# openai/procgen

Hardware: NVIDIA H100
Metric: env-steps/sec (higher is better)
Workload: dtype f32+u8

## Files before the change

procgen_b200/csrc/pg_kernels.cuh:

```cuda
#pragma once
#include "pg_raster.cuh"

namespace pg {

struct KParams {
    EnvHdr *hdr;
    Entity *ents;
    int16_t *grid;
    MT19937 *rng;
    MT19937 *lvl_rng;
    int32_t *scratch;
    RotBlit *rot_scratch;
    Blit *blit_list;
    unsigned char *frame_setup;
    Blit *cell_spill;
    const GameAssets *assets;
    const uint32_t *atlas;
    TileTable tiles;
    const int32_t *action;
    uint8_t *rgb;
    float *rew;
    uint8_t *first;
    int32_t *info_prev_level_seed;
    uint8_t *info_prev_level_complete;
// ... 115 lines not shown
}

template <class G, class Setup>
PG_HD void env_setup_frame(const KParams &p, int env, Setup &f, int lane, int nlanes) {
    Ctx c = make_ctx(p, env);
    using R = Raster<G, Setup>;
    R::setup_frame(c, f, p.snap != 0, lane, nlanes);
#if defined(__CUDA_ARCH__)
    __syncwarp();
#endif
    R::build_entity_blits(c, f, lane, nlanes);
#if defined(__CUDA_ARCH__)
    __syncwarp();
#endif
    if (f.n_jobs > 0) {
        R::frame_tiles(c, f, lane, nlanes);
#if defined(__CUDA_ARCH__)
        __syncwarp();
#endif
    }
    if (G::DEFER_ROTATED) {
        R::frame_rots(c, f, lane, nlanes);
#if defined(__CUDA_ARCH__)
        __syncwarp();
#endif
    }
    if (lane == 0)
        R::frame_append_overlays(f);
    if (G::DRAWS_GRID) {
#if defined(__CUDA_ARCH__)
        __syncwarp();
#endif
        R::frame_build(c, f, lane, nlanes, 0);
#if defined(__CUDA_ARCH__)
        __syncwarp();
#endif
        R::frame_tile_alloc(c, f, p.tiles, lane, nlanes);
#if defined(__CUDA_ARCH__)
        __syncwarp();
#endif
        R::frame_cells_finish(c, f, lane, nlanes);
    } else {
        R::frame_build(c, f, lane, nlanes, 0);
    }
}

template <class Frame>
PG_HD void env_stage_tiles_serial(const KParams &p, Frame &f) {
    const int nj = f.n_tjobs < MAX_TILE_JOBS ? f.n_tjobs : MAX_TILE_JOBS;
    for (int j = 0; j < nj; j++)
        for (int w = 0; w < (int)f.tjob_words[j]; w++) f.arena[f.tjob_dst[j] + w] = p.tiles.texels[f.tjob_src[j] + w];
}

template <class G, class Frame>
PG_HD void env_render_compose(const KParams &p, Frame &f, int row_first, int row_step, int lane, int nlanes) {
    Raster<G, Frame>::compose_rows(f, f.fb, row_first, row_step, lane, nlanes, p.atlas);
}

PG_HD void tile_table_fill(const SpriteDesc *sprites, const uint32_t *index, uint32_t *texels, const uint32_t *atlas, int slot, int tw, int th, int tid,
                           int nthreads) {
    Blit b;
    make_image_blit(b, 0.0, 0.0, (double)tw, (double)th, sprites[slot], false, 256, true);
    uint32_t *dst = texels + index[(slot * MAX_TILE_DIM + (tw - 1)) * MAX_TILE_DIM + (th - 1)];
    const int words = tile_words(tw, th);
    for (int i = tid; i < words; i += nthreads) {
        const int dy = i / tw, dx = i - dy * tw;
        dst[i] = dy < th ? tile_texel(b, atlas, dx, dy) : 0u;
    }
}

template <class G, int VIEW = G::MAX_VIEW_CELLS>
struct FrameFor {
    using type = FrameT<(G::DRAWS_GRID ? VIEW : 1), G::MAX_VISIBLE_ENTS, G::MAX_ROT_BLITS>;
    using setup = FrameSetupT<(G::DRAWS_GRID ? VIEW : 1), G::MAX_VISIBLE_ENTS, G::MAX_ROT_BLITS>;
    using shared = typename type::Shared;
};

}
```

procgen_b200/csrc/pg_launch.cuh:

```cuda
#pragma once
#include <stdarg.h>
#include <stdio.h>
#include <stdlib.h>
#include <string.h>

#include "pg_kernels.cuh"

#ifndef PG_HOSTSIM
#include <cuda_runtime.h>
#endif

namespace pg {

static inline void pg_fatal(const char *fmt, ...) {
    fprintf(stderr, "fatal: ");
    va_list args;
    va_start(args, fmt);
    vfprintf(stderr, fmt, args);
    va_end(args);
    exit(EXIT_FAILURE);
}
#define pg_fassert(cond)                                                                  \
    do {                                                                                  \
        if (!(cond)) {                                                                    \
// ... 104 lines not shown
    }
}
__device__ __forceinline__ void pg_bulk_load(void *dst_smem, const void *src_gmem, unsigned bytes, unsigned long long *bar) {
    asm volatile("cp.async.bulk.shared::cluster.global.mbarrier::complete_tx::bytes [%0], [%1], %2, [%3];" ::"r"(pg_smem_addr(dst_smem)),
                 "l"(src_gmem), "r"(bytes), "r"(pg_smem_addr(bar))
                 : "memory");
}
__device__ __forceinline__ void pg_bulk_store_and_wait(void *dst_gmem, const void *src_smem, unsigned bytes) {
    asm volatile("cp.async.bulk.global.shared::cta.bulk_group [%0], [%1], %2;" ::"l"(dst_gmem), "r"(pg_smem_addr(src_smem)), "r"(bytes) : "memory");
    asm volatile("cp.async.bulk.commit_group;" ::: "memory");
    asm volatile("cp.async.bulk.wait_group.read 0;" ::: "memory");
}

template <class G, int VIEW>
__global__ void __launch_bounds__(kRenderThreads, RenderTune<G, VIEW>::kMinBlocks) render_kernel(KParams p) {
    using Frame = typename FrameFor<G, VIEW>::type;
    extern __shared__ __align__(128) unsigned char smem_raw[];
    Frame &f = *reinterpret_cast<Frame *>(smem_raw);
    const int env = p.env_first + (int)blockIdx.x * p.env_step;
    const int tid = (int)threadIdx.x;
#ifdef PG_PHASE_TIMING
    long long t0 = clock64(), t1;
#define PG_RENDER_PHASE(id)                                       \
    do {                                                          \
        t1 = clock64();                                           \
        if (tid == 0)                                             \
            p.hdr[env].dbg_phase[id] = (uint32_t)(t1 - t0);       \
        t0 = t1;                                                  \
    } while (0)
#else
#define PG_RENDER_PHASE(id) do { } while (0)
#endif
    using Shared = typename FrameFor<G, VIEW>::shared;
    using Setup = typename FrameFor<G, VIEW>::setup;
    const Setup *gs = reinterpret_cast<const Setup *>(p.frame_setup + (size_t)env * p.frame_setup_stride);
    if (tid == 0)
        pg_mbar_init(&f.mbar, 1);
    __syncthreads();
    if (tid < 32) {
        const int nj = G::DRAWS_GRID ? (gs->n_tjobs < MAX_TILE_JOBS ? gs->n_tjobs : MAX_TILE_JOBS) : 0;
        unsigned words = 0;
        for (int j = tid; j < nj; j += 32) words += gs->tjob_words[j];
        for (int d = 16; d > 0; d >>= 1) words += __shfl_xor_sync(0xffffffffu, words, d);
        if (tid == 0) {
            pg_mbar_arrive_expect_tx(&f.mbar, (unsigned)sizeof(Shared) + 4u * words);
            pg_bulk_load(static_cast<Shared *>(&f), static_cast<const Shared *>(gs), (unsigned)sizeof(Shared), &f.mbar);
        }
        __syncwarp();
        for (int j = tid; j < nj; j += 32)
            pg_bulk_load(f.arena + gs->tjob_dst[j], p.tiles.texels + gs->tjob_src[j], 4u * gs->tjob_words[j], &f.mbar);
    }
    pg_mbar_wait(&f.mbar, 0);
    PG_RENDER_PHASE(0);
    env_render_compose<G, Frame>(p, f, tid >> 5, kRenderThreads >> 5, tid & 31, 32);
    __syncthreads();
    PG_RENDER_PHASE(5);
    if (p.consumer != nullptr) {
        const int kf = p.consumer_k, s = p.consumer_slot;
        const int slots = kf == 1 ? 1 : 2 * kf;
        uint32_t *base = reinterpret_cast<uint32_t *>(p.consumer) + (size_t)env * slots * (3 * RES_W * RES_H / 2);
        const uint16_t *lut = p.consumer_lut;
        for (int pair = tid; pair < RES_W * RES_H / 2; pair += kRenderThreads) {
            const uint32_t c0 = f.fb[2 * pair], c1 = f.fb[2 * pair + 1];
#pragma unroll
            for (int ch = 0; ch < 3; ch++) {
                const int sh = 16 - 8 * ch;
                const uint32_t v = (uint32_t)lut[(c0 >> sh) & 0xffu] | ((uint32_t)lut[(c1 >> sh) & 0xffu] << 16);
                base[(size_t)(s * 3 + ch) * (RES_W * RES_H / 2) + pair] = v;
                if (kf > 1)
                    base[(size_t)((s + kf) * 3 + ch) * (RES_W * RES_H / 2) + pair] = v;
            }
        }
        if (kf > 1 && p.first[env]) {
            for (int j = 1; j < kf; j++) {
                const int a = (s + j) % kf;
                for (int w = tid; w < 3 * RES_W * RES_H / 2; w += kRenderThreads) {
                    base[(size_t)a * (3 * RES_W * RES_H / 2) + w] = 0u;
                    base[(size_t)(a + kf) * (3 * RES_W * RES_H / 2) + w] = 0u;
                }
            }
        }
    }
    {
        constexpr int kQuadsPerThread = RES_W * RES_H / 4 / kRenderThreads;
        uint32_t c[kQuadsPerThread][4];
#pragma unroll
        for (int j = 0; j < kQuadsPerThread; j++) {
            const uint4 v = reinterpret_cast<const uint4 *>(f.fb)[tid + j * kRenderThreads];
            c[j][0] = v.x; c[j][1] = v.y; c[j][2] = v.z; c[j][3] = v.w;
        }
        __syncthreads();
#pragma unroll
        for (int j = 0; j < kQuadsPerThread; j++) Raster<G, Frame>::pack_quad(c[j], f.fb + 3 * (tid + j * kRenderThreads));
    }
    asm volatile("fence.proxy.async.shared::cta;" ::: "memory");
    __syncthreads();
    PG_RENDER_PHASE(6);
    if (tid == 0)
        pg_bulk_store_and_wait(p.rgb + (size_t)env * (RES_W * RES_H * 3), f.fb, RES_W * RES_H * 3);
    PG_RENDER_PHASE(7);
#undef PG_RENDER_PHASE
}

#endif

#ifndef PG_HOSTSIM
template <class G>
__global__ void camera_kernel(KParams p) {
    using Frame = typename FrameFor<G>::type;
    if (threadIdx.x == 0 && blockIdx.x < (unsigned)p.env_count) {
        const int env = p.env_first + (int)blockIdx.x * p.env_step;
        Ctx c = make_ctx(p, env);
        Raster<G, Frame>::prepare_camera(c);
        write_step_outputs(p, env, *c.h);
    }
}
#endif

template <class G, int VIEW, class Frame>
void render_env_serial(const KParams &p, int env, Frame &f) {
    using Setup = typename FrameFor<G, VIEW>::setup;
    using Shared = typename FrameFor<G, VIEW>::shared;
    Setup &s = *reinterpret_cast<Setup *>(p.frame_setup + (size_t)env * p.frame_setup_stride);
    env_setup_frame<G, Setup>(p, env, s, 0, 1);
    static_cast<Shared &>(f) = static_cast<const Shared &>(s);
    env_stage_tiles_serial<Frame>(p, f);
    for (int w = 0; w < 4; w++) env_render_compose<G, Frame>(p, f, w, 4, 0, 1);
    uint32_t *out = reinterpret_cast<uint32_t *>(p.rgb + (size_t)env * (RES_W * RES_H * 3));
    for (int g = 0; g < RES_W * RES_H / 4; g++) Raster<G, Frame>::pack_quad(f.fb + 4 * g, out + 3 * g);
}

struct LaunchCtx {
#ifndef PG_HOSTSIM
    cudaStream_t stream;
    cudaStream_t logic_stream;
    cudaEvent_t link;
    unsigned int *ticket;
    int max_logic_blocks;
    int render_smem_floor;
    cudaEvent_t *tev;
#endif
    int64_t *launch_counter;
};

#ifndef PG_HOSTSIM
template <class G, int VIEW>
int prepare_render_smem(const LaunchCtx &lc) {
    using Frame = typename FrameFor<G, VIEW>::type;
    const int bytes = (int)sizeof(Frame) > lc.render_smem_floor ? (int)sizeof(Frame) : lc.render_smem_floor;
    static int attr_set[64] = {};
    int dev = 0;
    CUDA_CHECK(cudaGetDevice(&dev));
    int &have = attr_set[dev & 63];
    if (have < bytes) {
        CUDA_CHECK(cudaFuncSetAttribute(render_kernel<G, VIEW>, cudaFuncAttributeMaxDynamicSharedMemorySize, bytes));
        have = bytes;
    }
    return bytes;
}
#endif

template <class G, bool INIT, int VIEW>
void launch_env_kernel(const KParams &p, const LaunchCtx &lc) {
    using Frame = typename FrameFor<G, VIEW>::type;
    if (p.env_count <= 0)
        return;
#ifndef PG_HOSTSIM
    const int render_smem = prepare_render_smem<G, VIEW>(lc);
    int logic_blocks = (p.env_count + kLogicEnvsPerBlock - 1) / kLogicEnvsPerBlock;
    if (logic_blocks > lc.max_logic_blocks)
        logic_blocks = lc.max_logic_blocks;
    cudaStream_t ls = lc.logic_stream ? lc.logic_stream : lc.stream;
    CUDA_CHECK(cudaMemsetAsync(lc.ticket, 0, sizeof(unsigned int), ls));
    if (lc.tev)
        CUDA_CHECK(cudaEventRecord(lc.tev[0], ls));
    logic_kernel<G, INIT><<<logic_blocks, kLogicThreads, 0, ls>>>(p, lc.ticket);
    if (lc.logic_stream) {
        CUDA_CHECK(cudaEventRecord(lc.link, ls));
        CUDA_CHECK(cudaStreamWaitEvent(lc.stream, lc.link, 0));
    }
// ... 97 lines not shown
```

procgen_b200/csrc/pg_raster.cuh:

```cuda
#pragma once
#include "pg_engine.cuh"

namespace pg {

enum BlitKind : uint8_t { BLIT_NONE = 0, BLIT_IMAGE = 1, BLIT_SOLID = 2, BLIT_ROTATED = 3, BLIT_SPANS = 4,
                          BLIT_ROT_PENDING = 5  };

struct Blit {
    uint8_t x1, y1, w, h;
    uint8_t kind;
    uint8_t mirror;
    uint16_t opacity;
    int32_t ix, iy;
    uint32_t basex, srcy;
    uint32_t src;
    uint16_t sw, sh;
};
static_assert(sizeof(Blit) == 32, "Blit is 32 B");

struct RotBlit {
    uint8_t x1[RES_H], x2[RES_H];
    int32_t absolute;
    int32_t dudx, dvdx, dudy, dvdy, u0, v0;
    int32_t pad;
    double m11, m12, m21, m22, dx, dy;
};

constexpr int MAX_BG_BLITS = 8;
constexpr int MAX_OVERLAY_BLITS = 8;

struct Camera {
    float unit, view_dim, x_off, y_off;
};

constexpr int MAX_TILE_DIM = 12;
constexpr int TILE_VARIANTS = MAX_TILE_DIM * MAX_TILE_DIM;
struct TileTable {
    const uint32_t *texels;
    const uint32_t *index;
    const SpriteDesc *sprites;
    int32_t n_slots;
};
PG_HD int tile_words(int tw, int th) { return (tw * th + 3) & ~3; }

constexpr int CELL_KEY_TYPES = 64;
constexpr int CELL_KEYS = CELL_KEY_TYPES * 4;
constexpr uint16_t CELL_GENERAL = 0x8000u;
constexpr int MAX_TILE_JOBS = 64;
constexpr uint32_t BG_NONE = 0xffffffffu;

constexpr uint32_t CI_BASE_MASK = 0xfffu;
constexpr uint32_t CI_VALID = 1u << 12;
constexpr int CI_D_SHIFT = 13;
constexpr int CI_TW_SHIFT = 18;
constexpr uint32_t CI_MULTI = 1u << 23;
constexpr uint32_t CI_FAST = 1u << 24;

template <int MAX_CELLS_1D, int MAX_ENT_BLITS, int MAX_ROT_BLITS>
struct alignas(16) FrameSharedT {
    static constexpr int kMaxCells1D = MAX_CELLS_1D;
    static constexpr int kMaxRot = MAX_ROT_BLITS > 0 ? MAX_ROT_BLITS : 1;
    static constexpr int kMaxEntBlits = MAX_ENT_BLITS;
    static constexpr int kMaxList = MAX_ENT_BLITS + MAX_OVERLAY_BLITS;
    static constexpr int kArenaWords = MAX_CELLS_1D > 1 ? (MAX_CELLS_1D * MAX_CELLS_1D * 8 < 1280 ? MAX_CELLS_1D * MAX_CELLS_1D * 8 : 1280) : 4;
    Camera cam;
    int32_t low_x, low_y, nx, ny;
    int32_t n_bg, n_ent, n_ent_below, n_overlay;
    int32_t snap;
    int32_t pad;
    int32_t tile_w0, tile_h0;
    int32_t n_rot;
    int32_t n_gen;
    int32_t tile_top;
    int32_t n_tjobs;
    RotBlit *rot;
    Blit *ents;
    Blit *gen_spill;
    int32_t n_strip_cols;
    int32_t spare;
    double cell_w;
    double spare_d;
    double col_x[MAX_CELLS_1D];
    double row_y[MAX_CELLS_1D];
    static constexpr int kSpanBytes = (MAX_CELLS_1D + 3) & ~3;
    alignas(4) uint8_t col_p1[kSpanBytes];
    alignas(4) uint8_t col_p2[kSpanBytes];
    alignas(4) uint8_t row_p1[kSpanBytes];
    alignas(4) uint8_t row_p2[kSpanBytes];
    uint8_t col_tw[MAX_CELLS_1D], row_th[MAX_CELLS_1D];
    uint8_t col_k0[MAX_CELLS_1D], row_k0[MAX_CELLS_1D];
    uint8_t strip_cols[RES_W];
    uint8_t col_lo[RES_W], col_hi[RES_W];
    uint8_t row_lo[RES_H], row_hi[RES_H];
    alignas(4) uint32_t colinfo[RES_W];
    uint32_t rowinfo[RES_H];
    uint32_t bgrow[RES_H];
    uint32_t tjob_src[MAX_TILE_JOBS];
    uint16_t tjob_dst[MAX_TILE_JOBS], tjob_words[MAX_TILE_JOBS];
    uint16_t cellmap[MAX_CELLS_1D * MAX_CELLS_1D];
    alignas(16) Blit bg[MAX_BG_BLITS];

    PG_HD Blit *gen_blit(int k) { return gen_spill + k; }
    PG_HD const Blit *gen_blit(int k) const { return gen_spill + k; }
};

template <int MAX_CELLS_1D, int MAX_ENT_BLITS, int MAX_ROT_BLITS>
struct alignas(16) FrameSetupT : FrameSharedT<MAX_CELLS_1D, MAX_ENT_BLITS, MAX_ROT_BLITS> {
    using Shared = FrameSharedT<MAX_CELLS_1D, MAX_ENT_BLITS, MAX_ROT_BLITS>;
    static constexpr int kMaxTileJobs = 64;
    int32_t n_jobs;
    int32_t job_ei[kMaxTileJobs], job_pos[kMaxTileJobs], job_n[kMaxTileJobs], job_j0[kMaxTileJobs];
    Blit overlay[MAX_OVERLAY_BLITS];
    alignas(4) uint16_t tilekey[MAX_CELLS_1D > 1 ? CELL_KEYS : 4];
};

template <int MAX_CELLS_1D, int MAX_ENT_BLITS, int MAX_ROT_BLITS>
struct alignas(16) FrameT : FrameSharedT<MAX_CELLS_1D, MAX_ENT_BLITS, MAX_ROT_BLITS> {
    using Shared = FrameSharedT<MAX_CELLS_1D, MAX_ENT_BLITS, MAX_ROT_BLITS>;
    alignas(16) uint32_t fb[RES_W * RES_H];
    alignas(16) uint32_t arena[Shared::kArenaWords];
    alignas(8) unsigned long long mbar;
};

PG_HD void blit_clear(Blit &b) {
    b.x1 = b.y1 = b.w = b.h = 0;
    b.kind = BLIT_NONE;
}

#ifndef PG_SETUP_INLINE_BLIT
#define PG_SETUP_INLINE_BLIT 1
#endif
PG_HD void make_image_blit_inl(Blit &b, double tx, double ty, double tw, double th, SpriteDesc sd, bool mirror, int int_opacity, bool snap);
PG_HD_FREE_NOINLINE void make_image_blit(Blit &b, double tx, double ty, double tw, double th, SpriteDesc sd, bool mirror, int int_opacity, bool snap) {
    make_image_blit_inl(b, tx, ty, tw, th, sd, mirror, int_opacity, snap);
}
PG_HD void make_image_blit_inl(Blit &b, double tx, double ty, double tw, double th, SpriteDesc sd, bool mirror, int int_opacity, bool snap) {
    blit_clear(b);
    const int sw = sd.w, sh = sd.h;
    if (sw <= 0 || sh <= 0)
        return;
    if (snap) {
        double x = pg_qround(tx);
        double y = pg_qround(ty);
        double w = pg_qround(tx + tw - x);
        double h = pg_qround(ty + th - y);
        tx = x;
        ty = y;
        tw = w;
        th = h;
    }
    if (tw == 0 || th == 0 || tw != tw || th != th)
        return;
    const double sx = (double)sw / tw;
    const double sy = (double)sh / th;
    const int ix = (int)(65536.0 * sx);
    const int iy = (int)(65536.0 * sy);
    double nx = tx, ny = ty, nw = tw, nh = th;
    if (nw < 0) { nx += nw; nw = -nw; }
    if (nh < 0) { ny += nh; nh = -nh; }
    int tx1 = pg_qround(nx), ty1 = pg_qround(ny);
    int tx2 = pg_qround(nx + nw), ty2 = pg_qround(ny + nh);
    if (tx1 < 0) tx1 = 0;
    if (ty1 < 0) ty1 = 0;
    if (tx2 > RES_W) tx2 = RES_W;
    if (ty2 > RES_H) ty2 = RES_H;
    if (tx2 <= tx1 || ty2 <= ty1)
        return;
    int h = ty2 - ty1;
    int w = tx2 - tx1;
    int dstx, dsty;
    if (sx < 0)
        dstx = (int)pg_dfloor((tx1 + 0.5 - (tx + tw)) * sx * 65536) + 1 + sw * 65536;
    else
// ... 904 lines not shown
    static PG_HD void span_of(double t, double tw, bool snap, int limit, uint8_t &p1, uint8_t &p2, uint8_t &tile_size, uint8_t &clip) {
        tile_size = 0;
        clip = 0;
        if (snap) {
            double x = pg_qround(t);
            tw = pg_qround(t + tw - x);
            t = x;
            if (tw >= 1 && tw <= MAX_TILE_DIM && x > -tw) {
                tile_size = (uint8_t)(int)tw;
                clip = x < 0 ? (uint8_t)(int)(-x) : 0;
            }
        }
        int a = pg_qround(t), b2 = pg_qround(t + tw);
        if (a < 0) a = 0;
        if (b2 > limit) b2 = limit;
        if (b2 < a) b2 = a;
        p1 = (uint8_t)a;
        p2 = (uint8_t)b2;
    }

    static PG_HD void setup_frame(Ctx &c, Frame &f, bool snap, int tid, int nthreads) {
        EnvHdr &h = *c.h;
        const Camera cam = camera_of(h);
        int low_x, low_y, nx, ny;
        grid_window(h, low_x, low_y, nx, ny);
        if (!G::DRAWS_GRID) {
            if (h.options.center_agent)
                h.err |= ERR_UNSUPPORTED;
            nx = 0;
            ny = 0;
        }
        bool overflow = false;
        if (nx > Frame::kMaxCells1D) { nx = Frame::kMaxCells1D; overflow = true; }
        if (ny > Frame::kMaxCells1D) { ny = Frame::kMaxCells1D; overflow = true; }
        double cw[4];
        screen_rect(cam, 0.f, 1.f, 1, 1, RENDER_EPS, cw);
        const int w0 = (int)pg_dfloor(cw[2]);
        if (tid == 0) {
            f.cam = cam;
            f.snap = snap ? 1 : 0;
            f.low_x = low_x;
            f.low_y = low_y;
            f.nx = nx;
            f.ny = ny;
            f.n_overlay = 0;
            f.n_bg = 0;
            f.n_ent = 0;
            f.n_ent_below = 0;
            f.n_rot = 0;
            f.n_jobs = 0;
            f.n_gen = 0;
            f.tile_top = 0;
            f.n_tjobs = 0;
            f.n_strip_cols = 0;
            f.tile_w0 = f.tile_h0 = w0;
            f.cell_w = cw[2];
            f.rot = reinterpret_cast<RotBlit *>(c.rot_scratch_raw);
            f.ents = c.blit_list;
            f.gen_spill = c.cell_spill;
            if (overflow)
                h.err |= ERR_BLIT_OVERFLOW;
            if (h.options.use_backgrounds)
                G::make_background_blits(c, f);
            f.pad = 0;
            if (f.n_bg == 1) {
                const Blit &b0 = f.bg[0];
                if (b0.kind == BLIT_IMAGE && b0.opacity == 256 && !b0.mirror)
                    f.pad = 1;
            }
            if (h.has_useful_vel_info && h.options.paint_vel_info) {
                const Entity &a = agent_of(c);
                const float infodim = (float)(RES_H * .2);
                float f1 = (float)(.5 * (double)a.vx / (double)h.maxspeed + .5);
                float f2 = (float)(.5 * (double)a.vy / (double)h.max_jump + .5);
                int s1 = (int)(f1 * 255), s2 = (int)(f2 * 255);
                s1 = s1 < 0 ? 0 : (s1 > 255 ? 255 : s1);
                s2 = s2 < 0 ? 0 : (s2 > 255 ? 255 : s2);
                make_solid_blit(f.overlay[0], 0, 0, (double)infodim, (double)infodim, ((uint32_t)s1 << 16) | ((uint32_t)s1 << 8) | (uint32_t)s1);
                make_solid_blit(f.overlay[1], (double)infodim, 0, (double)infodim, (double)infodim,
                                ((uint32_t)s2 << 16) | ((uint32_t)s2 << 8) | (uint32_t)s2);
                f.n_overlay = 2;
            }
            G::make_overlay_blits(c, f);
        }
        if (G::DRAWS_GRID) {
            uint32_t *keys = reinterpret_cast<uint32_t *>(f.tilekey);
            for (int i = tid; i < CELL_KEYS / 2; i += nthreads) keys[i] = 0;
        }
        for (int i = tid; i < nx; i += nthreads) {
            double r[4];
            screen_rect(cam, (float)(low_x + i), (float)(low_y + 1), 1, 1, RENDER_EPS, r);
            f.col_x[i] = r[0];
            uint8_t ts;
            span_of(r[0], r[2], snap, RES_W, f.col_p1[i], f.col_p2[i], ts, f.col_k0[i]);
            f.col_tw[i] = (ts == w0 || ts == w0 + 1) ? ts : 0;
        }
        for (int jj = tid; jj < ny; jj += nthreads) {
            int j = ny - 1 - jj;
            double r[4];
            screen_rect(cam, (float)low_x, (float)(low_y + j + 1), 1, 1, RENDER_EPS, r);
            f.row_y[j] = r[1];
            uint8_t ts;
            span_of(r[1], r[3], snap, RES_H, f.row_p1[j], f.row_p2[j], ts, f.row_k0[j]);
            f.row_th[j] = (ts == w0 || ts == w0 + 1) ? ts : 0;
        }
        for (int i = nx + tid; i < Frame::kSpanBytes; i += nthreads) f.col_p1[i] = f.col_p2[i] = 255;
        for (int j = ny + tid; j < Frame::kSpanBytes; j += nthreads) f.row_p1[j] = f.row_p2[j] = 255;
// ... 249 lines not shown
                    }
                }
                count += total;
#if defined(__CUDA_ARCH__)
                if (multi_warp)
                    __syncthreads();
#endif
            }
            if (z == -1)
                below = count;
        }
        if (count > Frame::kMaxEntBlits)
            count = Frame::kMaxEntBlits;
        if (below > count)
            below = count;
        if (tid == 0) {
            if (!G::ENTS_BELOW_GRID && below > 0)
                c.h->err |= ERR_UNSUPPORTED;
            f.n_ent = count;
            f.n_ent_below = below;
            if (count > c.h->max_blits_seen)
                c.h->max_blits_seen = count;
            if (f.n_rot > c.h->max_rots_seen)
                c.h->max_rots_seen = f.n_rot;
        }
    }

    static PG_HD bool clipped_walk_matches(int s, int t, int k0) {
        if (k0 == 0)
            return true;
        const double sx = (double)s / (double)t;
        const int ix = (int)(65536.0 * sx);
        const uint32_t bu = (uint32_t)((int)pg_dceil((0 + 0.5 - 0.0) * sx * 65536) - 1);
        const uint32_t bc = (uint32_t)((int)pg_dceil((0 + 0.5 - (double)(-k0)) * sx * 65536) - 1);
        for (int j = 0; j + k0 < t; j++)
            if (((bc + (uint32_t)ix * (uint32_t)j) >> 16) != ((bu + (uint32_t)ix * (uint32_t)(j + k0)) >> 16))
                return false;
        return true;
    }

    static PG_HD void frame_build(Ctx &c, Frame &f, int tid, int nthreads, int ) {
        const int wtid = tid, wn = nthreads;
        if (f.pad == 1) {
            const Blit &b = f.bg[0];
            for (int py = wtid; py < RES_H; py += wn) {
                const uint32_t dy = (uint32_t)py - b.y1;
                f.bgrow[py] = dy < b.h ? b.src + ((b.srcy + (uint32_t)b.iy * dy) >> 16) * b.sw : BG_NONE;
            }
        }
        if (!G::DRAWS_GRID)
            return;
        for (int px = wtid; px < RES_W + RES_H; px += wn) {
            if (px < RES_W) {
                const uint32_t w = cell_lookup(f.col_p1, f.col_p2, f.col_tw, f.col_k0, f.nx, f.ny, px, f.col_lo[px], f.col_hi[px]);
                f.colinfo[px] = w;
                if (w & CI_MULTI) {
                    int slot;
#if defined(__CUDA_ARCH__)
                    slot = atomicAdd(&f.n_strip_cols, 1);
#else
                    slot = f.n_strip_cols++;
#endif
                    f.strip_cols[slot] = (uint8_t)px;
                }
            } else {
                f.rowinfo[px - RES_W] = cell_lookup(f.row_p1, f.row_p2, f.row_th, f.row_k0, f.ny, 1, px - RES_W, f.row_lo[px - RES_W], f.row_hi[px - RES_W]);
            }
        }
        const int ncells = f.nx * f.ny;
        const bool mono = c.h->options.use_monochrome_assets != 0;
#if defined(__CUDA_ARCH__)
        for (int j = wtid; j < f.ny; j += wn) {
            const int gy = f.low_y + j, gx = f.low_x < 0 ? 0 : f.low_x;
            if (gy >= 0 && gy < c.mh && gx < c.mw) {
                const int16_t *row = c.grid + gy * c.mw + gx;
                asm volatile("prefetch.global.L1 [%0];" ::"l"(row));
                if (f.nx > 32 || ((reinterpret_cast<uintptr_t>(row) & 127) + 2 * f.nx > 128))
                    asm volatile("prefetch.global.L1 [%0];" ::"l"(row + f.nx - 1 < c.grid + c.mh * c.mw ? row + f.nx - 1 : row));
            }
        }
#endif
        int ci = f.ny > 0 ? wtid / f.ny : 0, cj = wtid - ci * f.ny;
        for (int k = wtid; k < ncells; k += wn) {
            if (k != wtid) {
                cj += wn;
                while (cj >= f.ny) {
                    cj -= f.ny;
                    ci++;
                }
            }
            f.cellmap[k] = 0;
            if (f.col_p1[ci] >= f.col_p2[ci] || f.row_p1[cj] >= f.row_p2[cj])
                continue;
            int type = E::get_obj(c, f.low_x + ci, f.low_y + cj);
            if (type == INVALID_OBJ)
                continue;
            const int img_type = G::image_for_type(c, type);
            if (img_type < 0 || img_type == SPACE)
                continue;
            const int theme = G::theme_for_grid_obj(c, type);
            const int tw = f.col_tw[ci], th = f.row_th[cj];
            if (tw && th && !mono && type >= 0 && type < CELL_KEY_TYPES && theme >= 0 && theme < MAX_IMAGE_THEMES) {
                double adj[4];
                bool ok = img_type >= 0 && img_type < USE_ASSET_THRESHOLD && !G::get_adjusted_image_rect(c, img_type, adj);
                if (ok && (f.col_k0[ci] | f.row_k0[cj])) {
                    const int masked_theme = (c.h->options.restrict_themes && !G::should_preserve_type_themes(c, img_type)) ? 0 : theme;
                    const SpriteDesc sd = c.assets->sprites[img_type + masked_theme * MAX_ASSETS];
                    ok = sd.w != 0 && clipped_walk_matches(sd.w, tw, f.col_k0[ci]) && clipped_walk_matches(sd.h, th, f.row_k0[cj]);
                }
                if (ok) {
                    const int key = type * 4 + (tw - f.tile_w0) + 2 * (th - f.tile_h0);
                    f.tilekey[key] = 1;
                    f.cellmap[k] = (uint16_t)(0x4000 | key);
                    continue;
                }
            }
            int slot;
// ... 76 lines not shown
            const int ci = k / f.ny, cj = k - ci * f.ny;
            const int type = key >> 2;
            Blit b;
            double r[4] = {f.col_x[ci], f.row_y[cj], f.cell_w, f.cell_w};
            make_sprite_blit(c, f, b, r, 0, false, type, G::theme_for_grid_obj(c, type), 1.0f);
            if (b.kind == BLIT_NONE)
                continue;
            *f.gen_blit(slot) = b;
            f.cellmap[k] = (uint16_t)(CELL_GENERAL | slot);
        }
    }

    static PG_HD void frame_tiles(Ctx &c, Frame &f, int tid, int nthreads) {
        const int nj = f.n_jobs < Frame::kMaxTileJobs ? f.n_jobs : Frame::kMaxTileJobs;
        for (int job = 0; job < nj; job++) {
            const int ei = f.job_ei[job], pos = f.job_pos[job], nt = f.job_n[job], j0 = f.job_j0[job];
            for (int j = tid; j < nt; j += nthreads) entity_tile_blit(c, f, ei, j0 + j, f.ents[pos + j]);
        }
    }

    static PG_HD void frame_rots(Ctx &c, Frame &f, int tid, int nthreads) {
        const int n = f.n_ent;
        for (int i = tid; i < n; i += nthreads) {
            if (f.ents[i].kind != BLIT_ROT_PENDING)
                continue;
            const int ei = (int)f.ents[i].src;
            const Entity &o = c.ents[ei];
            double r[4];
            object_rect(f.cam, o, r);
            Blit nb;
            make_sprite_blit(c, f, nb, r, o.rotation, o.is_reflected != 0, o.image_type, o.image_theme, o.alpha);
            f.ents[i] = nb;
        }
    }

    static PG_HD void frame_append_overlays(Frame &f) {
        for (int i = 0; i < f.n_overlay; i++) f.ents[f.n_ent + i] = f.overlay[i];
    }

    static PG_HD int ctz64(uint64_t m) {
#if defined(__CUDA_ARCH__)
        return __ffsll((long long)m) - 1;
#else
        return __builtin_ctzll(m);
#endif
    }
    static PG_HD int top_bit64(uint64_t m) {
#if defined(__CUDA_ARCH__)
        return 63 - __clzll((long long)m);
#else
        return 63 - __builtin_clzll(m);
#endif
    }


    static PG_HD uint32_t cell_layer(const Frame &f, uint32_t code, int ci, int cj, int px, int py, const uint32_t *atlas) {
        if (code & CELL_GENERAL)
            return blit_texel(*f.gen_blit((int)(code & 0x7fffu)), px, py, atlas, f.rot);
        const int dx = px - f.col_p1[ci] + f.col_k0[ci], dy = py - f.row_p1[cj] + f.row_k0[cj];
        return f.arena[(int)code - 1 + dy * f.col_tw[ci] + dx];
    }

    static PG_HD uint32_t bg_column(const Frame &f, int px) {
        const Blit &b = f.bg[0];
        const uint32_t dx = (uint32_t)px - b.x1;
        return dx < b.w ? (b.basex + (uint32_t)b.ix * dx) >> 16 : BG_NONE;
    }
    static PG_HD uint32_t bg_single(uint32_t bgrow, uint32_t bgcol, const uint32_t *atlas) {
        return (bgrow != BG_NONE && bgcol != BG_NONE) ? atlas[bgrow + bgcol] : 0xff000000u;
    }
    static PG_HD_NOINLINE uint32_t bg_generic(const Frame &f, int px, int py, const uint32_t *atlas) {
        uint32_t dst = 0xff000000u;
        if (f.pad == 1)
            return bg_single(f.bgrow[py], bg_column(f, px), atlas);
        for (int i = 0; i < f.n_bg; i++) dst = layer_over(dst, blit_texel(f.bg[i], px, py, atlas, f.rot));
        return dst;
    }

    static PG_HD uint32_t cells_over(const Frame &f, int px, int py, const uint32_t *atlas, uint32_t under) {
        uint32_t dst = under;
        const int clo = f.col_lo[px], chi = f.col_hi[px], rlo = f.row_lo[py], rhi = f.row_hi[py];
        if (clo != 255 && rlo != 255) {
            for (int ci = clo; ci <= chi; ci++)
                for (int cj = rlo; cj <= rhi; cj++) {
                    const uint32_t code = f.cellmap[ci * f.ny + cj];
                    if (code && px >= f.col_p1[ci] && px < f.col_p2[ci] && py >= f.row_p1[cj] && py < f.row_p2[cj])
                        dst = layer_over(dst, cell_layer(f, code, ci, cj, px, py, atlas));
                }
        }
        return dst;
    }
    static PG_HD_NOINLINE uint32_t cells_generic(const Frame &f, int px, int py, const uint32_t *atlas, uint32_t under) {
        return cells_over(f, px, py, atlas, under);
    }

    struct QuadCtx {
        uint32_t ci[4];
        uint32_t cbase[4];
        uint32_t tile_dx[4], tile_tw[4];
        uint32_t bg_sx[4];
        bool bg_one;
    };
    static PG_HD void quad_begin(const Frame &f, int px0, QuadCtx &q) {
        q.bg_one = f.pad == 1;
        for (int k = 0; k < 4; k++) {
            const uint32_t ci = G::DRAWS_GRID ? f.colinfo[px0 + k] : 0u;
            q.ci[k] = ci;
            q.cbase[k] = ci & CI_BASE_MASK;
            q.tile_dx[k] = (ci >> CI_D_SHIFT) & 31u;
            q.tile_tw[k] = (ci >> CI_TW_SHIFT) & 31u;
            q.bg_sx[k] = q.bg_one ? bg_column(f, px0 + k) : 0u;
        }
    }

    enum GatherMode { GATHER_ALL = 0, GATHER_BG = 1, GATHER_CELLS = 2 };

    template <int MODE>
    static PG_HD void gather_quad(const Frame &f, const QuadCtx &q, int px0, int py, const uint32_t *atlas, uint32_t *fb) {
        const uint32_t rowinfo = (G::DRAWS_GRID && MODE != GATHER_BG) ? f.rowinfo[py] : 0u;
        const uint32_t bgrow = q.bg_one ? f.bgrow[py] : BG_NONE;
        const uint32_t rbase = rowinfo & CI_BASE_MASK, dy = (rowinfo >> CI_D_SHIFT) & 31u;
        uint32_t *dst = fb + py * RES_W + px0;
        uint32_t s[4];
        uint32_t slow = 0, strip = 0;
        for (int k = 0; k < 4; k++) {
            s[k] = 0;
            if (G::DRAWS_GRID && MODE != GATHER_BG) {
                const uint32_t both = q.ci[k] & rowinfo;
                if (both & CI_FAST) {
                    const uint32_t code = f.cellmap[q.cbase[k] + rbase];
                    if (code & CELL_GENERAL) {
                        const Blit &gb = *f.gen_blit((int)(code & 0x7fffu));
                        if (gb.kind == BLIT_SOLID) {
                            const uint32_t box = *reinterpret_cast<const uint32_t *>(&gb);
                            const uint32_t ddx = (uint32_t)(px0 + k) - (box & 0xffu), ddy = (uint32_t)py - ((box >> 8) & 0xffu);
                            s[k] = (ddx < ((box >> 16) & 0xffu) && ddy < (box >> 24)) ? gb.src : 0u;
                        } else {
                            slow |= 1u << k;
                        }
                    } else if (code) {
                        s[k] = f.arena[code - 1 + dy * q.tile_tw[k] + q.tile_dx[k]];
                    }
                } else if (both & CI_VALID) {
                    strip |= 1u << k;
                }
            }
        }
        uint32_t c[4];
        for (int k = 0; k < 4; k++) {
            c[k] = s[k];
            if ((strip >> k) & 1u)
                continue;
            if (s[k] >= 0xff000000u && !((slow >> k) & 1u))
                continue;
            uint32_t under;
            if (MODE == GATHER_CELLS)
                under = dst[k];
            else if (q.bg_one)
                under = bg_single(bgrow, q.bg_sx[k], atlas);
            else
                under = bg_generic(f, px0 + k, py, atlas);
            if ((slow >> k) & 1u)
                c[k] = cells_generic(f, px0 + k, py, atlas, under);
            else
                c[k] = s[k] != 0 ? s[k] + pg_byte_mul(under, (~s[k]) >> 24) : under;
        }
        if (MODE == GATHER_CELLS) {
            for (int k = 0; k < 4; k++)
                if (!((strip >> k) & 1u))
                    dst[k] = c[k];
        } else {
#if defined(__CUDA_ARCH__)
            *reinterpret_cast<uint4 *>(dst) = make_uint4(c[0], c[1], c[2], c[3]);
#else
            for (int k = 0; k < 4; k++) dst[k] = c[k];
#endif
        }
    }

    template <int MODE>
    static PG_HD void gather_strips(const Frame &f, uint32_t *fb, int row_first, int row_step, int lane, int nlanes, const uint32_t *atlas) {
        const int my_rows = (RES_H - row_first + row_step - 1) / row_step;
        const int n1 = f.n_strip_cols * my_rows;
        for (int idx = lane; idx < n1; idx += nlanes) {
            const int px = f.strip_cols[idx / my_rows], py = row_first + (idx % my_rows) * row_step;
            if (!(f.rowinfo[py] & CI_VALID))
                continue;
            uint32_t *dst = fb + py * RES_W + px;
            const uint32_t under = MODE == GATHER_CELLS ? *dst : bg_generic(f, px, py, atlas);
            *dst = cells_over(f, px, py, atlas, under);
        }
        for (int r = 0; r < my_rows; r++) {
            const int py = row_first + r * row_step;
            if (!(f.rowinfo[py] & CI_MULTI))
                continue;
            for (int px = lane; px < RES_W; px += nlanes) {
                const uint32_t ci = f.colinfo[px];
                if (!(ci & CI_VALID) || (ci & CI_MULTI))
                    continue;
                uint32_t *dst = fb + py * RES_W + px;
                const uint32_t under = MODE == GATHER_CELLS ? *dst : bg_generic(f, px, py, atlas);
                *dst = cells_over(f, px, py, atlas, under);
            }
        }
    }

    static PG_HD void paint_blits(const Frame &f, uint32_t *fb, int lo, int hi, int row_first, int row_step, int lane, int nlanes, const uint32_t *atlas) {
        for (int i = lo; i < hi; i++) {
            const Blit &b = f.ents[i];
            const uint32_t box = *reinterpret_cast<const uint32_t *>(&b);
            const int x1 = (int)(box & 0xffu), y1 = (int)((box >> 8) & 0xffu), w = (int)((box >> 16) & 0xffu), h = (int)(box >> 24);
            if (w == 0)
                continue;
            int r0 = (row_first - y1) % row_step;
            if (r0 < 0)
                r0 += row_step;
            const int nrows = r0 < h ? (h - 1 - r0) / row_step + 1 : 0;
            const int n = nrows * w;
            const bool plain = b.kind == BLIT_IMAGE;
            for (int idx = lane; idx < n; idx += nlanes) {
                const int r = idx / w, dx = idx - r * w, dy = r0 + r * row_step;
                uint32_t s;
                if (plain) {
                    uint32_t sx = (b.basex + (uint32_t)b.ix * (uint32_t)dx) >> 16;
                    const uint32_t sy = (b.srcy + (uint32_t)b.iy * (uint32_t)dy) >> 16;
                    if (b.mirror)
                        sx = b.sw - 1 - sx;
                    s = layer_of(atlas[b.src + sy * b.sw + sx], b.opacity);
                } else {
                    s = blit_texel(b, x1 + dx, y1 + dy, atlas, f.rot);
                }
                if (s != 0) {
                    uint32_t *px = fb + (y1 + dy) * RES_W + x1 + dx;
                    *px = layer_over(*px, s);
                }
            }
#if defined(__CUDA_ARCH__)
            __syncwarp();
#endif
        }
    }

    static PG_HD void pack_quad(const uint32_t *c, uint32_t *out) {
#if defined(__CUDA_ARCH__)
        out[0] = __byte_perm(c[0], c[1], 0x6012);
        out[1] = __byte_perm(c[1], c[2], 0x5601);
        out[2] = __byte_perm(c[2], c[3], 0x4560);
#else
        const uint32_t r0 = (c[0] >> 16) & 0xff, g0 = (c[0] >> 8) & 0xff, b0 = c[0] & 0xff;
        const uint32_t r1 = (c[1] >> 16) & 0xff, g1 = (c[1] >> 8) & 0xff, b1 = c[1] & 0xff;
        const uint32_t r2 = (c[2] >> 16) & 0xff, g2 = (c[2] >> 8) & 0xff, b2 = c[2] & 0xff;
        const uint32_t r3 = (c[3] >> 16) & 0xff, g3 = (c[3] >> 8) & 0xff, b3 = c[3] & 0xff;
        out[0] = r0 | (g0 << 8) | (b0 << 16) | (r1 << 24);
        out[1] = g1 | (b1 << 8) | (r2 << 16) | (g2 << 24);
        out[2] = b2 | (r3 << 8) | (g3 << 16) | (b3 << 24);
#endif
    }

    static PG_HD void compose_rows(const Frame &f, uint32_t *fb, int row_first, int row_step, int lane, int nlanes, const uint32_t *atlas) {
        const int nb = f.n_ent_below, n_all = f.n_ent + f.n_overlay;
        const int per_row = RES_W / 4;
        const int sub = nlanes >= per_row ? nlanes / per_row : 1;
        for (int qx = lane % per_row; qx < per_row; qx += (nlanes < per_row ? nlanes : per_row)) {
            QuadCtx q;
            quad_begin(f, qx * 4, q);
            const int first = row_first + row_step * (nlanes >= per_row ? lane / per_row : 0);
            if (G::ENTS_BELOW_GRID && nb > 0) {
                for (int py = first; py < RES_H; py += row_step * sub) gather_quad<GATHER_BG>(f, q, qx * 4, py, atlas, fb);
            } else {
                for (int py = first; py < RES_H; py += row_step * sub) gather_quad<GATHER_ALL>(f, q, qx * 4, py, atlas, fb);
            }
        }
        if (G::DRAWS_GRID && !(G::ENTS_BELOW_GRID && nb > 0))
            gather_strips<GATHER_ALL>(f, fb, row_first, row_step, lane, nlanes, atlas);
        if (G::ENTS_BELOW_GRID && nb > 0) {
#if defined(__CUDA_ARCH__)
            __syncwarp();
#endif
            paint_blits(f, fb, 0, nb, row_first, row_step, lane, nlanes, atlas);
            for (int qx = lane % per_row; qx < per_row; qx += (nlanes < per_row ? nlanes : per_row)) {
                QuadCtx q;
                quad_begin(f, qx * 4, q);
                const int first = row_first + row_step * (nlanes >= per_row ? lane / per_row : 0);
                for (int py = first; py < RES_H; py += row_step * sub) gather_quad<GATHER_CELLS>(f, q, qx * 4, py, atlas, fb);
            }
            if (G::DRAWS_GRID)
                gather_strips<GATHER_CELLS>(f, fb, row_first, row_step, lane, nlanes, atlas);
        }
#if defined(__CUDA_ARCH__)
        __syncwarp();
#endif
        paint_blits(f, fb, (G::ENTS_BELOW_GRID ? nb : 0), n_all, row_first, row_step, lane, nlanes, atlas);
    }
};

template <class G>
struct DrawDefaults {
    template <class Frame>
    static PG_HD void make_background_blits(Ctx &c, Frame &f) {
        EnvHdr &h = *c.h;
        double main_rect[4];
        Raster<G, Frame>::screen_rect(f.cam, 0, (float)h.main_height, (float)h.main_width, (float)h.main_height, 0, main_rect);
        SpriteDesc bg = c.assets->backgrounds[h.background_index];
        if (h.bg_tile_ratio < 0) {
            const int nt = Raster<G, Frame>::tile_count(main_rect, h.bg_tile_ratio);
            int n = 0;
            for (int i = 0; i < nt; i++) {
                double tr[4];
                Raster<G, Frame>::tile_rect(main_rect, h.bg_tile_ratio, nt, i, tr);
                Blit b;
                make_image_blit(b, tr[0], tr[1], tr[2], tr[3], bg, false, 256, f.snap != 0);
                if (b.kind == BLIT_NONE)
                    continue;
                if (n < MAX_BG_BLITS)
                    f.bg[n++] = b;
                else
                    h.err |= ERR_BLIT_OVERFLOW;
            }
            f.n_bg = n;
            return;
        }
        float bgw = bg.w;
        float bgh = bg.h;
        float bg_ar = bgw / bgh;
        float world_ar = (float)(h.main_width * 1.0 / h.main_height);
        float extra_w = bg_ar - world_ar;
        float offset_x = h.bg_pct_x * extra_w;
        double adj[4] = {(double)(-offset_x), 0, (double)(bg_ar / world_ar), 1};
        Raster<G, Frame>::adjust_rect(main_rect, adj);
        make_image_blit(f.bg[0], main_rect[0], main_rect[1], main_rect[2], main_rect[3], bg, false, 256, f.snap != 0);
        f.n_bg = 1;
    }
    template <class Frame>
    static PG_HD void make_overlay_blits(Ctx &c, Frame &f) {}
    template <class Frame>
    static PG_HD bool make_grid_obj_blit(Ctx &c, const Frame &f, Blit &b, double *rect, int type, int theme) {
        if (!c.h->options.use_monochrome_assets)
            return false;
        if (c.h->options.restrict_themes && !G::should_preserve_type_themes(c, type))
            theme = 0;
        const int k = 4;
// ... 16 lines not shown
```

Before: 19.59 million.

## Replace strip-column gather with per-row slow-pixel bitmasks and branchless quad gather

Drops the atomically built strip-column list. Instead it computes per-row 64-bit masks of the pixels that need the slow path, using warp ballots over colinfo. The fast gather is now branchless: it renders two rows per call when the background is single, writes full quads with vector stores, and defers general cells by OR-ing bits into the mask. A compacted exceptions pass then walks the set bits with popc/fns to handle only those pixels. This aims to cut divergence and wasted lanes in strip handling, at the cost of an extra shared array, shared-memory atomics, and more warp syncs.

```diff
diff --git a/procgen_b200/csrc/pg_kernels.cuh b/procgen_b200/csrc/pg_kernels.cuh
--- a/procgen_b200/csrc/pg_kernels.cuh
+++ b/procgen_b200/csrc/pg_kernels.cuh
@@ -191,9 +191,9 @@
         for (int w = 0; w < (int)f.tjob_words[j]; w++) f.arena[f.tjob_dst[j] + w] = p.tiles.texels[f.tjob_src[j] + w];
 }
 
-template <class G, class Frame>
-PG_HD void env_render_compose(const KParams &p, Frame &f, int row_first, int row_step, int lane, int nlanes) {
-    Raster<G, Frame>::compose_rows(f, f.fb, row_first, row_step, lane, nlanes, p.atlas);
+template <class G, class Frame, class Gathered>
+PG_HD void env_render_compose(const KParams &p, Frame &f, int row_first, int row_step, int lane, int nlanes, Gathered gathered) {
+    Raster<G, Frame>::compose_rows(f, f.fb, row_first, row_step, lane, nlanes, p.atlas, gathered);
 }
 
 PG_HD void tile_table_fill(const SpriteDesc *sprites, const uint32_t *index, uint32_t *texels, const uint32_t *atlas, int slot, int tw, int th, int tid,
diff --git a/procgen_b200/csrc/pg_launch.cuh b/procgen_b200/csrc/pg_launch.cuh
--- a/procgen_b200/csrc/pg_launch.cuh
+++ b/procgen_b200/csrc/pg_launch.cuh
@@ -180,9 +180,9 @@
     }
     pg_mbar_wait(&f.mbar, 0);
     PG_RENDER_PHASE(0);
-    env_render_compose<G, Frame>(p, f, tid >> 5, kRenderThreads >> 5, tid & 31, 32);
+    env_render_compose<G, Frame>(p, f, tid >> 5, kRenderThreads >> 5, tid & 31, 32, [&] { PG_RENDER_PHASE(1); });
     __syncthreads();
-    PG_RENDER_PHASE(5);
+    PG_RENDER_PHASE(2);
     if (p.consumer != nullptr) {
         const int kf = p.consumer_k, s = p.consumer_slot;
         const int slots = kf == 1 ? 1 : 2 * kf;
@@ -223,10 +223,10 @@
     }
     asm volatile("fence.proxy.async.shared::cta;" ::: "memory");
     __syncthreads();
-    PG_RENDER_PHASE(6);
+    PG_RENDER_PHASE(3);
     if (tid == 0)
         pg_bulk_store_and_wait(p.rgb + (size_t)env * (RES_W * RES_H * 3), f.fb, RES_W * RES_H * 3);
-    PG_RENDER_PHASE(7);
+    PG_RENDER_PHASE(4);
 #undef PG_RENDER_PHASE
 }
 
@@ -253,7 +253,7 @@
     env_setup_frame<G, Setup>(p, env, s, 0, 1);
     static_cast<Shared &>(f) = static_cast<const Shared &>(s);
     env_stage_tiles_serial<Frame>(p, f);
-    for (int w = 0; w < 4; w++) env_render_compose<G, Frame>(p, f, w, 4, 0, 1);
+    for (int w = 0; w < 4; w++) env_render_compose<G, Frame>(p, f, w, 4, 0, 1, [] {});
     uint32_t *out = reinterpret_cast<uint32_t *>(p.rgb + (size_t)env * (RES_W * RES_H * 3));
     for (int g = 0; g < RES_W * RES_H / 4; g++) Raster<G, Frame>::pack_quad(f.fb + 4 * g, out + 3 * g);
 }
diff --git a/procgen_b200/csrc/pg_raster.cuh b/procgen_b200/csrc/pg_raster.cuh
--- a/procgen_b200/csrc/pg_raster.cuh
+++ b/procgen_b200/csrc/pg_raster.cuh
@@ -76,8 +76,6 @@
     RotBlit *rot;
     Blit *ents;
     Blit *gen_spill;
-    int32_t n_strip_cols;
-    int32_t spare;
     double cell_w;
     double spare_d;
     double col_x[MAX_CELLS_1D];
@@ -89,7 +87,6 @@
     alignas(4) uint8_t row_p2[kSpanBytes];
     uint8_t col_tw[MAX_CELLS_1D], row_th[MAX_CELLS_1D];
     uint8_t col_k0[MAX_CELLS_1D], row_k0[MAX_CELLS_1D];
-    uint8_t strip_cols[RES_W];
     uint8_t col_lo[RES_W], col_hi[RES_W];
     uint8_t row_lo[RES_H], row_hi[RES_H];
     alignas(4) uint32_t colinfo[RES_W];
@@ -119,6 +116,7 @@
     using Shared = FrameSharedT<MAX_CELLS_1D, MAX_ENT_BLITS, MAX_ROT_BLITS>;
     alignas(16) uint32_t fb[RES_W * RES_H];
     alignas(16) uint32_t arena[Shared::kArenaWords];
+    uint64_t slow_px[RES_H];
     alignas(8) unsigned long long mbar;
 };
 
@@ -1129,7 +1127,6 @@
             f.n_gen = 0;
             f.tile_top = 0;
             f.n_tjobs = 0;
-            f.n_strip_cols = 0;
             f.tile_w0 = f.tile_h0 = w0;
             f.cell_w = cw[2];
             f.rot = reinterpret_cast<RotBlit *>(c.rot_scratch_raw);
@@ -1485,17 +1482,7 @@
             return;
         for (int px = wtid; px < RES_W + RES_H; px += wn) {
             if (px < RES_W) {
-                const uint32_t w = cell_lookup(f.col_p1, f.col_p2, f.col_tw, f.col_k0, f.nx, f.ny, px, f.col_lo[px], f.col_hi[px]);
-                f.colinfo[px] = w;
-                if (w & CI_MULTI) {
-                    int slot;
-#if defined(__CUDA_ARCH__)
-                    slot = atomicAdd(&f.n_strip_cols, 1);
-#else
-                    slot = f.n_strip_cols++;
-#endif
-                    f.strip_cols[slot] = (uint8_t)px;
-                }
+                f.colinfo[px] = cell_lookup(f.col_p1, f.col_p2, f.col_tw, f.col_k0, f.nx, f.ny, px, f.col_lo[px], f.col_hi[px]);
             } else {
                 f.rowinfo[px - RES_W] = cell_lookup(f.row_p1, f.row_p2, f.row_th, f.row_k0, f.ny, 1, px - RES_W, f.row_lo[px - RES_W], f.row_hi[px - RES_W]);
             }
@@ -1678,6 +1665,23 @@
         return 63 - __builtin_clzll(m);
 #endif
     }
+    static PG_HD int popc64(uint64_t m) {
+#if defined(__CUDA_ARCH__)
+        return __popcll(m);
+#else
+        return __builtin_popcountll(m);
+#endif
+    }
+    static PG_HD int nth_bit64(uint64_t m, int n) {
+#if defined(__CUDA_ARCH__)
+        const uint32_t lo = (uint32_t)m;
+        const int nlo = __popc(lo);
+        return n < nlo ? (int)__fns(lo, 0u, n + 1) : 32 + (int)__fns((uint32_t)(m >> 32), 0u, n - nlo + 1);
+#else
+        for (; n > 0; n--) m &= m - 1;
+        return __builtin_ctzll(m);
+#endif
+    }
 
 
     static PG_HD uint32_t cell_layer(const Frame &f, uint32_t code, int ci, int cj, int px, int py, const uint32_t *atlas) {
@@ -1716,118 +1720,154 @@
         }
         return dst;
     }
-    static PG_HD_NOINLINE uint32_t cells_generic(const Frame &f, int px, int py, const uint32_t *atlas, uint32_t under) {
-        return cells_over(f, px, py, atlas, under);
-    }
-
     struct QuadCtx {
         uint32_t ci[4];
         uint32_t cbase[4];
         uint32_t tile_dx[4], tile_tw[4];
         uint32_t bg_sx[4];
-        bool bg_one;
     };
     static PG_HD void quad_begin(const Frame &f, int px0, QuadCtx &q) {
-        q.bg_one = f.pad == 1;
         for (int k = 0; k < 4; k++) {
             const uint32_t ci = G::DRAWS_GRID ? f.colinfo[px0 + k] : 0u;
             q.ci[k] = ci;
             q.cbase[k] = ci & CI_BASE_MASK;
             q.tile_dx[k] = (ci >> CI_D_SHIFT) & 31u;
             q.tile_tw[k] = (ci >> CI_TW_SHIFT) & 31u;
-            q.bg_sx[k] = q.bg_one ? bg_column(f, px0 + k) : 0u;
+            q.bg_sx[k] = f.pad == 1 ? bg_column(f, px0 + k) : 0u;
         }
     }
 
     enum GatherMode { GATHER_ALL = 0, GATHER_BG = 1, GATHER_CELLS = 2 };
 
+    static PG_HD void mark_strips(Frame &f, int row_first, int row_step, int lane, int nlanes) {
+        uint64_t cvalid = 0, cmulti = 0;
+#if defined(__CUDA_ARCH__)
+        for (int h = 0; h < RES_W; h += 32) {
+            const uint32_t ci = f.colinfo[h + lane];
+            cvalid |= (uint64_t)__ballot_sync(0xffffffffu, ci & CI_VALID) << h;
+            cmulti |= (uint64_t)__ballot_sync(0xffffffffu, ci & CI_MULTI) << h;
+        }
+#else
+        for (int px = 0; px < RES_W; px++) {
+            cvalid |= (uint64_t)((f.colinfo[px] & CI_VALID) != 0) << px;
+            cmulti |= (uint64_t)((f.colinfo[px] & CI_MULTI) != 0) << px;
+        }
+#endif
+        for (int py = row_first + lane * row_step; py < RES_H; py += nlanes * row_step) {
+            const uint32_t ri = f.rowinfo[py];
+            f.slow_px[py] = (ri & CI_MULTI) ? cvalid : (ri & CI_FAST) ? cmulti : 0ull;
+        }
+    }
+
+    template <int MODE, bool BG_ONE, int NR>
+    static PG_HD void gather_fast(Frame &f, const QuadCtx &q, int qx, int py0, int step, const uint32_t *atlas, uint32_t *fb) {
+        constexpr bool kCells = G::DRAWS_GRID && MODE != GATHER_BG;
+        uint32_t c[NR][4];
+        uint32_t slow[NR], gen[NR];
+        for (int r = 0; r < NR; r++) {
+            const int py = py0 + r * step;
+            const uint32_t ri = kCells ? f.rowinfo[py] : 0u;
+            const uint32_t rbase = ri & CI_BASE_MASK, dy = (ri >> CI_D_SHIFT) & 31u;
+            const uint32_t bgrow = BG_ONE ? f.bgrow[py] : BG_NONE;
+            const uint32_t *dst = fb + py * RES_W + qx * 4;
+            slow[r] = kCells ? (uint32_t)(f.slow_px[py] >> (qx * 4)) & 15u : 0u;
+            gen[r] = 0;
+            for (int k = 0; k < 4; k++) {
+                uint32_t s = 0;
+                if (kCells) {
+                    const uint32_t code = f.cellmap[q.cbase[k] + rbase];
+                    const bool single = (q.ci[k] & ri & CI_FAST) != 0;
+                    const bool tile = single && code - 1u < (uint32_t)CELL_GENERAL - 1u;
+                    gen[r] |= (single && (code & CELL_GENERAL)) ? 1u << k : 0u;
+                    const uint32_t t = f.arena[tile ? code - 1u + dy * q.tile_tw[k] + q.tile_dx[k] : 0u];
+                    s = tile ? t : 0u;
+                }
+                const bool opaque = s >= 0xff000000u;
+                uint32_t under;
+                if (MODE == GATHER_CELLS) {
+                    under = dst[k];
+                } else if (BG_ONE) {
+                    const bool fetch = !opaque && bgrow != BG_NONE && q.bg_sx[k] != BG_NONE;
+                    under = fetch ? atlas[bgrow + q.bg_sx[k]] : 0xff000000u;
+                } else {
+                    under = opaque ? 0u : bg_generic(f, qx * 4 + k, py, atlas);
+                }
+                c[r][k] = opaque ? s : (s != 0 ? s + pg_byte_mul(under, (~s) >> 24) : under);
+            }
+        }
+        for (int r = 0; r < NR; r++) {
+            const int py = py0 + r * step;
+            uint32_t *dst = fb + py * RES_W + qx * 4;
+            if ((slow[r] | gen[r]) == 0) {
+#if defined(__CUDA_ARCH__)
+                *reinterpret_cast<uint4 *>(dst) = make_uint4(c[r][0], c[r][1], c[r][2], c[r][3]);
+#else
+                for (int k = 0; k < 4; k++) dst[k] = c[r][k];
+#endif
+            } else {
+                for (int k = 0; k < 4; k++)
+                    if (!(((slow[r] | gen[r]) >> k) & 1u))
+                        dst[k] = c[r][k];
+                if (gen[r]) {
+#if defined(__CUDA_ARCH__)
+                    atomicOr(reinterpret_cast<unsigned long long *>(&f.slow_px[py]), (unsigned long long)gen[r] << (qx * 4));
+#else
+                    f.slow_px[py] |= (uint64_t)gen[r] << (qx * 4);
+#endif
+                }
+            }
+        }
+    }
+
     template <int MODE>
-    static PG_HD void gather_quad(const Frame &f, const QuadCtx &q, int px0, int py, const uint32_t *atlas, uint32_t *fb) {
-        const uint32_t rowinfo = (G::DRAWS_GRID && MODE != GATHER_BG) ? f.rowinfo[py] : 0u;
-        const uint32_t bgrow = q.bg_one ? f.bgrow[py] : BG_NONE;
-        const uint32_t rbase = rowinfo & CI_BASE_MASK, dy = (rowinfo >> CI_D_SHIFT) & 31u;
-        uint32_t *dst = fb + py * RES_W + px0;
-        uint32_t s[4];
-        uint32_t slow = 0, strip = 0;
-        for (int k = 0; k < 4; k++) {
-            s[k] = 0;
-            if (G::DRAWS_GRID && MODE != GATHER_BG) {
-                const uint32_t both = q.ci[k] & rowinfo;
-                if (both & CI_FAST) {
-                    const uint32_t code = f.cellmap[q.cbase[k] + rbase];
-                    if (code & CELL_GENERAL) {
-                        const Blit &gb = *f.gen_blit((int)(code & 0x7fffu));
-                        if (gb.kind == BLIT_SOLID) {
-                            const uint32_t box = *reinterpret_cast<const uint32_t *>(&gb);
-                            const uint32_t ddx = (uint32_t)(px0 + k) - (box & 0xffu), ddy = (uint32_t)py - ((box >> 8) & 0xffu);
-                            s[k] = (ddx < ((box >> 16) & 0xffu) && ddy < (box >> 24)) ? gb.src : 0u;
-                        } else {
-                            slow |= 1u << k;
-                        }
-                    } else if (code) {
-                        s[k] = f.arena[code - 1 + dy * q.tile_tw[k] + q.tile_dx[k]];
-                    }
-                } else if (both & CI_VALID) {
-                    strip |= 1u << k;
-                }
-            }
-        }
-        uint32_t c[4];
-        for (int k = 0; k < 4; k++) {
-            c[k] = s[k];
-            if ((strip >> k) & 1u)
-                continue;
-            if (s[k] >= 0xff000000u && !((slow >> k) & 1u))
-                continue;
-            uint32_t under;
-            if (MODE == GATHER_CELLS)
-                under = dst[k];
-            else if (q.bg_one)
-                under = bg_single(bgrow, q.bg_sx[k], atlas);
-            else
-                under = bg_generic(f, px0 + k, py, atlas);
-            if ((slow >> k) & 1u)
-                c[k] = cells_generic(f, px0 + k, py, atlas, under);
-            else
-                c[k] = s[k] != 0 ? s[k] + pg_byte_mul(under, (~s[k]) >> 24) : under;
-        }
-        if (MODE == GATHER_CELLS) {
-            for (int k = 0; k < 4; k++)
-                if (!((strip >> k) & 1u))
-                    dst[k] = c[k];
-        } else {
-#if defined(__CUDA_ARCH__)
-            *reinterpret_cast<uint4 *>(dst) = make_uint4(c[0], c[1], c[2], c[3]);
-#else
-            for (int k = 0; k < 4; k++) dst[k] = c[k];
-#endif
-        }
-    }
-
-    template <int MODE>
-    static PG_HD void gather_strips(const Frame &f, uint32_t *fb, int row_first, int row_step, int lane, int nlanes, const uint32_t *atlas) {
+    static PG_HD void gather_exceptions(const Frame &f, uint32_t *fb, int row_first, int row_step, int lane, int nlanes, const uint32_t *atlas) {
         const int my_rows = (RES_H - row_first + row_step - 1) / row_step;
-        const int n1 = f.n_strip_cols * my_rows;
-        for (int idx = lane; idx < n1; idx += nlanes) {
-            const int px = f.strip_cols[idx / my_rows], py = row_first + (idx % my_rows) * row_step;
-            if (!(f.rowinfo[py] & CI_VALID))
-                continue;
+        int r = -1, before = 0, n = 0;
+        uint64_t m = 0;
+        for (int e = lane;; e += nlanes) {
+            while (e >= before + n) {
+                before += n;
+                if (++r >= my_rows)
+                    return;
+                m = f.slow_px[row_first + r * row_step];
+                n = popc64(m);
+            }
+            const int px = nth_bit64(m, e - before), py = row_first + r * row_step;
             uint32_t *dst = fb + py * RES_W + px;
             const uint32_t under = MODE == GATHER_CELLS ? *dst : bg_generic(f, px, py, atlas);
             *dst = cells_over(f, px, py, atlas, under);
         }
-        for (int r = 0; r < my_rows; r++) {
-            const int py = row_first + r * row_step;
-            if (!(f.rowinfo[py] & CI_MULTI))
-                continue;
-            for (int px = lane; px < RES_W; px += nlanes) {
-                const uint32_t ci = f.colinfo[px];
-                if (!(ci & CI_VALID) || (ci & CI_MULTI))
-                    continue;
-                uint32_t *dst = fb + py * RES_W + px;
-                const uint32_t under = MODE == GATHER_CELLS ? *dst : bg_generic(f, px, py, atlas);
-                *dst = cells_over(f, px, py, atlas, under);
-            }
+    }
+
+    template <int MODE>
+    static PG_HD void gather_pass(Frame &f, uint32_t *fb, int row_first, int row_step, int lane, int nlanes, const uint32_t *atlas) {
+        constexpr bool kCells = G::DRAWS_GRID && MODE != GATHER_BG;
+        if (kCells) {
+            mark_strips(f, row_first, row_step, lane, nlanes);
+#if defined(__CUDA_ARCH__)
+            __syncwarp();
+#endif
+        }
+        constexpr int per_row = RES_W / 4;
+        const int step = row_step * (nlanes >= per_row ? nlanes / per_row : 1);
+        const int first = row_first + row_step * (nlanes >= per_row ? lane / per_row : 0);
+        for (int qx = lane % per_row; qx < per_row; qx += (nlanes < per_row ? nlanes : per_row)) {
+            QuadCtx q;
+            quad_begin(f, qx * 4, q);
+            int py = first;
+            if (f.pad == 1) {
+                for (; py + step < RES_H; py += 2 * step) gather_fast<MODE, true, 2>(f, q, qx, py, step, atlas, fb);
+                if (py < RES_H)
+                    gather_fast<MODE, true, 1>(f, q, qx, py, step, atlas, fb);
+            } else {
+                for (; py < RES_H; py += step) gather_fast<MODE, false, 1>(f, q, qx, py, step, atlas, fb);
+            }
+        }
+        if (kCells) {
+#if defined(__CUDA_ARCH__)
+            __syncwarp();
+#endif
+            gather_exceptions<MODE>(f, fb, row_first, row_step, lane, nlanes, atlas);
         }
     }
 
@@ -1883,36 +1923,20 @@
 #endif
     }
 
-    static PG_HD void compose_rows(const Frame &f, uint32_t *fb, int row_first, int row_step, int lane, int nlanes, const uint32_t *atlas) {
+    template <class Gathered>
+    static PG_HD void compose_rows(Frame &f, uint32_t *fb, int row_first, int row_step, int lane, int nlanes, const uint32_t *atlas, Gathered gathered) {
         const int nb = f.n_ent_below, n_all = f.n_ent + f.n_overlay;
-        const int per_row = RES_W / 4;
-        const int sub = nlanes >= per_row ? nlanes / per_row : 1;
-        for (int qx = lane % per_row; qx < per_row; qx += (nlanes < per_row ? nlanes : per_row)) {
-            QuadCtx q;
-            quad_begin(f, qx * 4, q);
-            const int first = row_first + row_step * (nlanes >= per_row ? lane / per_row : 0);
-            if (G::ENTS_BELOW_GRID && nb > 0) {
-                for (int py = first; py < RES_H; py += row_step * sub) gather_quad<GATHER_BG>(f, q, qx * 4, py, atlas, fb);
-            } else {
-                for (int py = first; py < RES_H; py += row_step * sub) gather_quad<GATHER_ALL>(f, q, qx * 4, py, atlas, fb);
-            }
-        }
-        if (G::DRAWS_GRID && !(G::ENTS_BELOW_GRID && nb > 0))
-            gather_strips<GATHER_ALL>(f, fb, row_first, row_step, lane, nlanes, atlas);
         if (G::ENTS_BELOW_GRID && nb > 0) {
+            gather_pass<GATHER_BG>(f, fb, row_first, row_step, lane, nlanes, atlas);
 #if defined(__CUDA_ARCH__)
             __syncwarp();
 #endif
             paint_blits(f, fb, 0, nb, row_first, row_step, lane, nlanes, atlas);
-            for (int qx = lane % per_row; qx < per_row; qx += (nlanes < per_row ? nlanes : per_row)) {
-                QuadCtx q;
-                quad_begin(f, qx * 4, q);
-                const int first = row_first + row_step * (nlanes >= per_row ? lane / per_row : 0);
-                for (int py = first; py < RES_H; py += row_step * sub) gather_quad<GATHER_CELLS>(f, q, qx * 4, py, atlas, fb);
-            }
-            if (G::DRAWS_GRID)
-                gather_strips<GATHER_CELLS>(f, fb, row_first, row_step, lane, nlanes, atlas);
-        }
+            gather_pass<GATHER_CELLS>(f, fb, row_first, row_step, lane, nlanes, atlas);
+        } else {
+            gather_pass<GATHER_ALL>(f, fb, row_first, row_step, lane, nlanes, atlas);
+        }
+        gathered();
 #if defined(__CUDA_ARCH__)
         __syncwarp();
 #endif
```

Result: no change. 19.63 million (median of 6 runs) (+0.2%).
